# G1OJS/PyFT8

Hardware: NVIDIA B200
Metric: decoded 15-s FT8 cycles/sec (higher is better)
Workload: dtype f32

## Files before the change

### pyft8_b200/csrc/fine.cuh

```cuda
#pragma once
#include <cuda_runtime.h>
#include <stdint.h>
#include "fft.cuh"
#include "sync.cuh"

namespace ft8 {

constexpr int CS_N = 96000, CS_N1 = 375, CS_N2 = 256, CS_COLS = 16, CS_NT = 256;
constexpr int FINE_SPEC_STRIDE = 49152;
constexpr int FINE_N = 3200, FINE_NT = 256;
#define FINE_BUFS 3
constexpr int FINE_NP = FINE_N + FINE_N / 200;

template <typename T> __device__ __forceinline__ float2 load_pair(const T* x, int n);
template <> __device__ __forceinline__ float2 load_pair<int16_t>(const int16_t* x, int n) {
    const short2 v = *reinterpret_cast<const short2*>(x + 2 * n);
    return make_float2((float)v.x, (float)v.y);
}
template <> __device__ __forceinline__ float2 load_pair<float>(const float* x, int n) {
    return *reinterpret_cast<const float2*>(x + 2 * n);
}

template <typename T>
__global__ void __launch_bounds__(CS_NT)
k_cs_cols(const T* __restrict__ audio, float2* __restrict__ Y, const float2* __restrict__ TC,
          const float2* __restrict__ W96000T) {
    extern __shared__ float2 cs_smem[];
    const int cyc = blockIdx.y, n2_0 = blockIdx.x * CS_COLS;
    const T* x = audio + (size_t)cyc * CYCLE_SAMPLES;
    constexpr int LD_ITERS = (CS_COLS * CS_N1 + CS_NT - 1) / CS_NT;
#pragma unroll
    for (int b0 = 0; b0 < LD_ITERS; b0 += 8) {
        float2 v[8];
#pragma unroll
        for (int u = 0; u < 8; ++u) {
            const int i = threadIdx.x + (b0 + u) * CS_NT;
            const int n1 = i / CS_COLS, c = i - n1 * CS_COLS;
            const int n = CS_N2 * n1 + n2_0 + c;
            v[u] = (i < CS_COLS * CS_N1 && n < CYCLE_SAMPLES / 2) ? load_pair<T>(x, n) : make_float2(0.f, 0.f);
        }
#pragma unroll
        for (int u = 0; u < 8; ++u) {
            const int i = threadIdx.x + (b0 + u) * CS_NT;
            const int n1 = i / CS_COLS, c = i - n1 * CS_COLS;
            if (i < CS_COLS * CS_N1) cs_smem[c * CS_N1 + n1] = v[u];
        }
    }
    __syncthreads();
    pass_inplace_batched<375, 3, 1, CS_COLS, CS_NT, false, true>(cs_smem, threadIdx.x, TC);
    pass_inplace_batched<375, 5, 3, CS_COLS, CS_NT, false, true, true>(cs_smem, threadIdx.x, TC + 250);
    pass_inplace_batched<375, 5, 15, CS_COLS, CS_NT, false, true>(cs_smem, threadIdx.x, TC + 350);
    pass_inplace_batched<375, 5, 75, CS_COLS, CS_NT, false>(cs_smem, threadIdx.x, TC);
    float2* y = Y + (size_t)cyc * CS_N;
    for (int i = threadIdx.x; i < CS_COLS * CS_N1; i += CS_NT) {
        const int k1 = i / CS_COLS, c = i - k1 * CS_COLS;
        const int n2 = n2_0 + c;
        const float2 w = __ldg(&W96000T[k1 * CS_N2 + n2]);
        y[k1 * CS_N2 + n2] = cmul(cs_smem[c * CS_N1 + k1], w);
    }
}

constexpr int CSR_G = 8;
constexpr int CSR_STRIDE = CS_N2 + CS_N2 / 16 + 4;
__global__ void __launch_bounds__(CS_NT)
k_cs_rows(const float2* __restrict__ Y, float2* __restrict__ spec, int spec_stride, int kmax,
          const float2* __restrict__ T256, const float2* __restrict__ W192000) {
    __shared__ float2 rows[2 * CSR_G][CSR_STRIDE];
    const int cyc = blockIdx.y, g0 = blockIdx.x * CSR_G;
    const float2* y = Y + (size_t)cyc * CS_N;
    {
        float2 v[2 * CSR_G];
#pragma unroll
        for (int r = 0; r < 2 * CSR_G; ++r) {
            const int k1 = g0 + (r & (CSR_G - 1));
            const int row = (r < CSR_G) ? k1 : (CS_N1 - k1) % CS_N1;
            v[r] = (k1 <= 187) ? y[row * CS_N2 + threadIdx.x] : make_float2(0.f, 0.f);
        }
#pragma unroll
        for (int r = 0; r < 2 * CSR_G; ++r) rows[r][threadIdx.x] = v[r];
    }
    __syncthreads();
    pass_inplace_batched<256, 16, 1, 2 * CSR_G, CS_NT, false, true, false, IdMap, Pad16Map, CSR_STRIDE>(&rows[0][0], threadIdx.x, T256);
    pass_inplace_batched<256, 16, 16, 2 * CSR_G, CS_NT, false, false, false, Pad16Map, IdMap, CSR_STRIDE>(&rows[0][0], threadIdx.x, T256);
    float2* out = spec + (size_t)cyc * spec_stride;
    for (int i = threadIdx.x; i < CSR_G * CS_N2; i += CS_NT) {
        const int k2 = i / CSR_G, r = i - k2 * CSR_G;
        const int k1 = g0 + r;
        if (k1 > 187) continue;
        const int k = k1 + CS_N1 * k2;
        const int k2m = (k1 == 0) ? ((CS_N2 - k2) & (CS_N2 - 1)) : (CS_N2 - 1 - k2);
        const float2 zk = rows[r][k2];
        const float2 zm = rows[CSR_G + r][k2m];
        const float2 e = cscale(0.5f, cfma_elem(zm, 1.0f, -1.0f, zk));
        const float2 dz = cfma_elem(zm, -1.0f, 1.0f, zk);
            const float2 o = make_float2(0.5f * dz.y, -0.5f * dz.x);
        const float2 wo = cmul(o, __ldg(&W192000[k]));
        if (k <= kmax) out[k] = cadd(e, wo);
        const int km = CS_N - k;
        if (km <= kmax && !(k1 == 0 && k2 > 128)) out[km] = make_float2(e.x - wo.x, -(e.y - wo.y));
    }
}

struct FineTables {
    float taper[100];
    float2 w32[32];
};
__constant__ FineTables c_fine;

struct FineOut {
    int32_t tt, ff, nsync;
    float sd;
    int32_t snr;
};

constexpr int FINE_T5_OFF = 4 * 640, FINE_T8_OFF = FINE_T5_OFF + 4 * 128, FINE_TF_LEN = FINE_T8_OFF + 7 * 16;

struct FineIn { float2 a0[5]; float2 ax[4]; };

__device__ __forceinline__ void fine_pass12_load(FineIn& in, const float2* __restrict__ spec, int fb, int p2) {
#pragma unroll
    for (int j = 0; j < 5; ++j) in.a0[j] = __ldg(&spec[fb + p2 + 128 * j]);
    in.ax[0] = __ldg(&spec[fb + p2 + 640]);
    in.ax[1] = (p2 + 128 < 210) ? __ldg(&spec[fb + p2 + 128 + 640]) : make_float2(0.f, 0.f);
    in.ax[2] = (p2 + 384 >= 490) ? __ldg(&spec[fb + p2 + 384 - 640]) : make_float2(0.f, 0.f);
    in.ax[3] = __ldg(&spec[fb + p2 + 512 - 640]);
}

template <int Q, bool A4> __device__ __forceinline__ float2 fine_b(float2 a0, float2 ax) {
    const float2 w1 = make_float2(0.30901699437494742410f, 0.95105651629515357212f);
    const float2 w2 = make_float2(-0.80901699437494742410f, 0.58778525229247312917f);
    if (Q == 0) return cadd(a0, ax);
    const float2 w = (Q == 1 || Q == 4) ? w1 : w2;
    const bool conj = (Q >= 3) != A4;
    return cadd(a0, conj ? cmulc(ax, w) : cmul(ax, w));
}

template <int Q>
__device__ __forceinline__ void fine_pass12_col(const FineIn& in, const float2 (&ax)[4], float2* dst, int p2,
                                                const float2* __restrict__ TF, const float2 (&w)[8]) {
    float2 a[5];
    a[0] = fine_b<Q, false>(in.a0[0], ax[0]);
    a[1] = (p2 < 82) ? fine_b<Q, false>(in.a0[1], ax[1]) : in.a0[1];
    a[2] = in.a0[2];
    a[3] = (p2 >= 106) ? fine_b<Q, true>(in.a0[3], ax[2]) : in.a0[3];
    a[4] = fine_b<Q, true>(in.a0[4], ax[3]);
    if (Q > 0) {
#pragma unroll
        for (int j = 0; j < 5; ++j) a[j] = cmulc(a[j], __ldg(&TF[(Q - 1) * 640 + p2 + 128 * j]));
    }
    Dft<5, true>::run(a);
    dst[Q + 25 * p2] = a[0];
#pragma unroll
    for (int k = 1; k < 5; ++k) dst[Q + 25 * p2 + 5 * k] = cmulc(a[k], w[k - 1]);
}

__device__ __forceinline__ void fine_pass12_finish(const FineIn& in, float2* dst, int p2, const float2* __restrict__ TF,
                                                   const float* taper, const float2 (&w)[8]) {
    float2 ax[4] = {in.ax[0], in.ax[1], in.ax[2], in.ax[3]};
    if (p2 >= 110) ax[0] = cscale(taper[p2 - 110], ax[0]);
    if (p2 < 82) ax[1] = cscale(taper[p2 + 18], ax[1]);
    if (p2 >= 106) ax[2] = cscale(taper[p2 - 106], ax[2]);
    if (p2 < 78) ax[3] = cscale(taper[p2 + 22], ax[3]);
    fine_pass12_col<0>(in, ax, dst, p2, TF, w);
    fine_pass12_col<1>(in, ax, dst, p2, TF, w);
    fine_pass12_col<2>(in, ax, dst, p2, TF, w);
    fine_pass12_col<3>(in, ax, dst, p2, TF, w);
    fine_pass12_col<4>(in, ax, dst, p2, TF, w);
}

__device__ __forceinline__ void fine_pass12(float2* dst, const float2* __restrict__ spec, int fb, int p2,
                                            const float2* __restrict__ TF, const float* taper, const float2 (&w)[8]) {
    FineIn in;
    fine_pass12_load(in, spec, fb, p2);
    fine_pass12_finish(in, dst, p2, TF, taper, w);
}

template <int NT>
__device__ __forceinline__ void fine_pass3(const float2* src, float2* dst, int tid, const float2 (&tw8)[7]) {
    const int p = tid & 15;
#pragma unroll
    for (int r = 0; r < (25 * 16 + NT - 1) / NT; ++r) {
        const int q = (tid >> 4) + (NT / 16) * r;
        if (q < 25) {
            float2 a[8];
#pragma unroll
            for (int j = 0; j < 8; ++j) a[j] = src[q + 25 * p + 400 * j];
            Dft<8, true>::run(a);
            float2* d = dst + q + 201 * p;
            d[0] = a[0];
#pragma unroll
            for (int k = 1; k < 8; ++k) d[25 * k] = cmulc(a[k], tw8[k - 1]);
        }
    }
    __syncthreads();
}

template <int NT>
__device__ __forceinline__ void fine_last_full(const float2* src, float2* dst, int tid) {
#pragma unroll
    for (int t0 = 0; t0 < 200; t0 += NT) {
        const int t = t0 + tid;
        if (t < 200) {
            float2 a[16];
#pragma unroll
            for (int j = 0; j < 16; ++j) a[j] = src[t + 201 * j];
            Dft<16, true>::run(a);
#pragma unroll
            for (int k = 0; k < 16; ++k) dst[t + 200 * k] = a[k];
        }
    }
    __syncthreads();
}

__device__ __forceinline__ void fine_pass4_window(const float2* x, float2* zwin, int n0, int len, int tid, const float2* w16) {
#pragma unroll
    for (int o = tid; o < 256; o += 128) if (o < len) {
        const int n = n0 + o;
        const int kk = n / 200, q = n - 200 * kk;
        const int r = kk & 3;
        const float sg = (r & 1) ? -1.0f : 1.0f;
        const float2 ir = make_float2(r == 0 ? 1.0f : (r == 2 ? -1.0f : 0.0f), r == 1 ? 1.0f : (r == 3 ? -1.0f : 0.0f));
        float2 y[4];
#pragma unroll
        for (int b = 0; b < 4; ++b) {
            const float2 x0 = x[q + 201 * b], x1 = x[q + 201 * (4 + b)], x2 = x[q + 201 * (8 + b)], x3 = x[q + 201 * (12 + b)];
            const float2 s = caxpy(sg, x2, x0), t = caxpy(sg, x3, x1);
            y[b] = cmac(s, t, ir);
        }
        float2 acc = y[0];
#pragma unroll
        for (int b = 1; b < 4; ++b) acc = cmac(acc, y[b], w16[(b * kk) & 15]);
        zwin[o] = acc;
    }
}

__device__ __forceinline__ float2 shfl_xor2(float2 v, int o) {
    return make_float2(__shfl_xor_sync(0xffffffffu, v.x, o), __shfl_xor_sync(0xffffffffu, v.y, o));
}

__device__ __forceinline__ float dft32x4_mag(const float2* z, int i0, int lane, const float2 (&tw)[8]) {
    const int m = lane & 7;
    float2 v[4];
#pragma unroll
    for (int a = 0; a < 4; ++a) v[a] = z[i0 + m + 8 * a];
    Dft<4, false>::run(v);
    float2 c[8];
#pragma unroll
    for (int t = 0; t < 8; ++t) c[t] = cmul(v[t & 3], tw[t]);
    const bool h4 = lane & 4, h2 = lane & 2, h1 = lane & 1;
    float2 d4[4], d2[2];
#pragma unroll
    for (int j = 0; j < 4; ++j) {
        const float2 send = h4 ? c[j] : c[j + 4], keep = h4 ? c[j + 4] : c[j];
        d4[j] = cadd(keep, shfl_xor2(send, 4));
    }
#pragma unroll
    for (int j = 0; j < 2; ++j) {
        const float2 send = h2 ? d4[j] : d4[j + 2], keep = h2 ? d4[j + 2] : d4[j];
        d2[j] = cadd(keep, shfl_xor2(send, 2));
    }
    const float2 send = h1 ? d2[0] : d2[1], keep = h1 ? d2[1] : d2[0];
    const float2 s = cadd(keep, shfl_xor2(send, 1));
    return sqrtf(fmaf(s.x, s.x, s.y * s.y)) * (1.0f / 3200.0f);
}

__device__ __forceinline__ int clip_start(int i) { return max(0, min(FINE_N - 32, i)); }

__device__ __forceinline__ float costas_rows4(const float2* z, int z0, int k0, int lane, const float2 (&tw)[8]) {
    const int k = k0 + (lane >> 3), bin = lane & 7;
    const float g = dft32x4_mag(z, z0 + 32 * min(k, 6), lane, tw);
    float c = 0.0f;
    if (k < 7 && bin < 7) c = (bin == ((0x2560413 >> (4 * k)) & 7)) ? g : g * (-1.0f / 6.0f);
#pragma unroll
    for (int o = 16; o > 0; o >>= 1) c += __shfl_xor_sync(0xffffffffu, c, o);
    return c;
}

constexpr int FINE_SMEM_BYTES = (FINE_N + 2 * FINE_NP) * (int)sizeof(float2) + (79 * 8 + 16 + 100) * (int)sizeof(float) + (32 + 16 + 256) * (int)sizeof(float2);

#ifdef FINE_PROFILE
__device__ unsigned long long g_fine_prof[16];
#define FP_T(v) const long long v = clock64()
#define FP_ADD(i, d) do { if (lane == 0) atomicAdd(&g_fine_prof[i], (unsigned long long)(d)); } while (0)
#else
#define FP_T(v)
#define FP_ADD(i, d)
#endif
__global__ void __launch_bounds__(FINE_NT, 2)
k_fine(const float2* __restrict__ spec, int spec_stride, const int32_t* __restrict__ list, const int32_t* __restrict__ count,
       int n_direct, const int32_t* __restrict__ cycle_of, const int16_t* __restrict__ cand_f0,
       const int16_t* __restrict__ cand_h0, const float2* __restrict__ TF, FineOut* __restrict__ fo,
       float* __restrict__ llr_fine, float* __restrict__ sig_grid) {
    extern __shared__ float2 fine_smem[];
    float* G = reinterpret_cast<float*>(fine_smem + FINE_N + 2 * FINE_NP);
    float* score = G + 79 * 8;
    float* taper = score + 16;
    float2* w32 = reinterpret_cast<float2*>(taper + 100);
    float2* w16 = w32 + 32;
    float2* zwin = w16 + 16;
    const int tid = threadIdx.x, lane = tid & 31, warp = tid >> 5;
    if (tid < 32) w32[tid] = c_fine.w32[tid];
    if (tid < 16) { const float2 w = c_fine.w32[2 * tid]; w16[tid] = make_float2(w.x, -w.y); }
    if (tid < 100) taper[tid] = c_fine.taper[tid];
    __syncthreads();
    float2 tw[8];
#pragma unroll
    for (int t = 0; t < 8; ++t) tw[t] = w32[(t * (lane & 7)) & 31];
    if (warp >= 4) {
#pragma unroll
        for (int k = 1; k < 5; ++k) tw[k - 1] = __ldg(&TF[FINE_T5_OFF + (k - 1) * 128 + (tid - 128)]);
    }
    float2 tw8[7];
#pragma unroll
    for (int k = 1; k < 8; ++k) tw8[k - 1] = __ldg(&TF[FINE_T8_OFF + (k - 1) * 16 + (tid & 15)]);
    const int n_items = list ? *count : n_direct;
    if (warp >= 4 && (int)blockIdx.x < n_items) {
        const int slot = list ? list[blockIdx.x] : (int)blockIdx.x;
        fine_pass12(fine_smem, spec + (size_t)cycle_of[slot] * spec_stride, 50 * cand_f0[slot], tid - 128, TF, taper, tw);
    }
    __syncthreads();
    for (int item = blockIdx.x; item < n_items; item += gridDim.x) {
        const int slot = list ? list[item] : item;
        const int cyc = cycle_of[slot];
        const int f0 = cand_f0[slot], h0 = cand_h0[slot];
        const float2* sp = spec + (size_t)cyc * spec_stride;
        const int fb0 = 50 * f0;
        const int tb0 = (h0 >= 0) ? 8 * h0 : 8 * h0 + 1;
        float2 *px = fine_smem, *po = fine_smem + FINE_N, *pb = fine_smem + FINE_N + FINE_NP;
        FineIn fin;
        FP_T(ts0);
        if (warp >= 4) fine_pass12_load(fin, sp, fb0 - 32, tid - 128);
        fine_pass3<FINE_NT>(px, po, tid, tw8);
        FP_T(ts1);
        if (warp < 4) {
            fine_pass4_window(po, zwin, tb0 - 8 + 1152, 238, tid, w16);
            asm volatile("bar.sync 1, 128;" ::: "memory");
#pragma unroll
            for (int u = 0; u < 2; ++u) {
                const int st = 2 * warp + u;
                const float sc = costas_rows4(zwin, 2 * st, 0, lane, tw) + costas_rows4(zwin, 2 * st, 4, lane, tw);
                if (lane == 0) score[st] = sc;
            }
            FP_T(ts2);
            if (warp == 0) { FP_ADD(8, ts1 - ts0); FP_ADD(9, ts2 - ts1); FP_ADD(11, 1); }
        } else {
            fine_pass12_finish(fin, px, tid - 128, TF, taper, tw);
            FP_T(ts2);
            if (warp == 4) FP_ADD(10, ts2 - ts1);
        }
        __syncthreads();
        int tt = -8;
        float bestf = score[0];
        for (int ti = 1; ti < 8; ++ti) if (score[ti] > bestf) { bestf = score[ti]; tt = -8 + 2 * ti; }
        { float2* t = pb; pb = po; po = t; }
        int best_fi = 4;
        for (int e = 0; e < 8; ++e) {
            const int fi = e < 4 ? e : e + 1;
            if (warp >= 4 && e < 7) fine_pass12_load(fin, sp, fb0 + (-32 + 8 * (e + 1 < 4 ? e + 1 : e + 2)), tid - 128);
            FP_T(t0);
            fine_pass3<FINE_NT>(px, po, tid, tw8);
            FP_T(t1);
            if (warp < 4) {
                fine_pass4_window(po, zwin, tb0 + tt + 1152, 224, tid, w16);
                FP_T(tw0);
                asm volatile("bar.sync 1, 128;" ::: "memory");
                if (warp < 2) {
                    const float r = costas_rows4(zwin, 0, 4 * warp, lane, tw);
                    if (lane == 0) score[8 + warp] = r;
                }
                FP_T(t2);
                if (warp == 0) { FP_ADD(0, t1 - t0); FP_ADD(1, t2 - t1); FP_ADD(4, tw0 - t1); FP_ADD(6, 1); }
                if (warp == 3) { FP_ADD(5, t2 - t1); }
            } else if (e < 7) {
                fine_pass12_finish(fin, px, tid - 128, TF, taper, tw);
                FP_T(t2);
                if (warp == 4) { FP_ADD(2, t2 - t1); FP_ADD(7, 1); }
            }
            __syncthreads();
            FP_T(t3);
            if (warp == 0) FP_ADD(3, t3 - t1);
            const float sc = score[8] + score[9];
            if (sc > bestf || (sc == bestf && fi < best_fi)) { bestf = sc; best_fi = fi; float2* t = pb; pb = po; po = t; }
        }
        const int ff = -32 + 8 * best_fi;
        FP_T(tf0);
        fine_last_full<FINE_NT>(pb, po, tid);
        FP_T(tf1);
        if (warp < 4) {
            const float2* z = po;
            for (int j0 = 4 * warp; j0 < 79; j0 += 16) {
                const int j = j0 + (lane >> 3);
                const float g = dft32x4_mag(z, clip_start(tb0 + tt + 32 * min(j, 78)), lane, tw);
                if (j < 79) G[j * 8 + (lane & 7)] = g;
            }
            asm volatile("bar.sync 1, 128;" ::: "memory");
            if (sig_grid) for (int i = tid; i < 79 * 8; i += 128) sig_grid[(size_t)slot * 632 + i] = G[i];
            if (tid < 32) {
                int hit = 0;
                if (lane < 21) {
                    const int blk = lane / 7, k = lane - 7 * blk;
                    const int row = (blk == 0) ? k : (blk == 1 ? 36 + k : 72 + k);
                    int am = 0;
                    float mv = G[row * 8];
                    for (int t = 1; t < 8; ++t) if (G[row * 8 + t] > mv) { mv = G[row * 8 + t]; am = t; }
                    hit = (am == ((0x2560413 >> (4 * k)) & 7)) ? 1 : 0;
                }
                const int nsync = __reduce_add_sync(0xffffffffu, hit);
                float p[2][8];
                if (lane < 29) {
#pragma unroll
                    for (int q = 0; q < 2; ++q) {
                        const int sym = lane + (q ? 43 : 7);
#pragma unroll
                        for (int t = 0; t < 8; ++t) p[q][t] = 20.0f * log10f(G[sym * 8 + t]);
                    }
                }
                float sd; int snr;
                llr_from_payload_warp(p, lane, llr_fine + (size_t)slot * 174, sd, snr);
                if (lane == 0) {
                    FineOut o; o.tt = tt; o.ff = ff; o.nsync = nsync; o.sd = sd; o.snr = snr;
                    fo[slot] = o;
// ... 20 lines not shown
```

### pyft8_b200/csrc/fine_tc.cuh

```cuda
#pragma once
#include <cuda_runtime.h>
#include <stdint.h>
#include "fine.cuh"

namespace ft8 {

struct TScanOut { int32_t tt; float score0; };

constexpr int FS_WIN = 224;
constexpr int FS_CAND = 32;
constexpr int FS_K1 = 64, FS_NU = 328, FS_K = FS_K1 + FS_NU, FS_KC = 8, FS_CHUNKS = FS_K / FS_KC;
constexpr int FS_N = 64;
constexpr int FS_TILES = 4;
constexpr int FS_STAGES = 4;
constexpr int FS_ACC_COLS = FS_TILES * FS_N;
constexpr int FS_A_STAGE_COLS = FS_TILES * 16;
constexpr int FS_B_SPLIT_BYTES = 2 * FS_N * 16;
constexpr int FS_B_STAGE_BYTES = 2 * FS_B_SPLIT_BYTES;
constexpr int FS_GEN_WARPS = 16;
constexpr int FS_BSTAGES = 8;
constexpr int FS_ISSUERS = 4;
constexpr int FS_NT = (FS_GEN_WARPS + FS_ISSUERS + 1) * 32;
constexpr int FS_W_LEN = 6400;
constexpr int FS_SMEM_BYTES = FS_BSTAGES * FS_B_STAGE_BYTES + FS_W_LEN * 8;
constexpr int FS_BMAT_FLOATS = FS_CHUNKS * FS_B_STAGE_BYTES / 4;
static_assert(FS_ACC_COLS + FS_STAGES * FS_A_STAGE_COLS == 512, "TMEM column plan");

__host__ __device__ __forceinline__ int fs_u_of(int j) { return j < 164 ? j - 182 : j + 554; }

__device__ __forceinline__ uint32_t smem_u32(const void* p) { return (uint32_t)__cvta_generic_to_shared(p); }
__device__ __forceinline__ void mbar_init(uint32_t a, int count) { asm volatile("mbarrier.init.shared::cta.b64 [%0], %1;" ::"r"(a), "r"(count)); }
__device__ __forceinline__ void mbar_expect_tx(uint32_t a, int bytes) {
    asm volatile("mbarrier.arrive.expect_tx.shared::cta.b64 _, [%0], %1;" ::"r"(a), "r"(bytes) : "memory");
}
__device__ __forceinline__ void mbar_wait(uint32_t a, uint32_t parity) {
    uint32_t done = 0;
    for (uint32_t spin = 0; !done; ++spin) {
        asm volatile("{\n\t.reg .pred p;\n\tmbarrier.try_wait.parity.shared::cta.b64 p, [%1], %2;\n\tselp.u32 %0, 1, 0, p;\n\t}"
                     : "=r"(done) : "r"(a), "r"(parity) : "memory");
        if (spin > (1u << 24)) __trap();
    }
}
__device__ __forceinline__ void bulk_g2s(uint32_t dst, const void* src, int bytes, uint32_t mbar) {
    asm volatile("cp.async.bulk.shared::cluster.global.mbarrier::complete_tx::bytes [%0], [%1], %2, [%3];"
                 ::"r"(dst), "l"(src), "r"(bytes), "r"(mbar) : "memory");
}
__device__ __forceinline__ void fence_proxy_async() { asm volatile("fence.proxy.async.shared::cta;" ::: "memory"); }
__device__ __forceinline__ void tc_fence_before() { asm volatile("tcgen05.fence::before_thread_sync;" ::: "memory"); }
__device__ __forceinline__ void tc_fence_after() { asm volatile("tcgen05.fence::after_thread_sync;" ::: "memory"); }
__device__ __forceinline__ void tc_commit(uint32_t mbar) {
    asm volatile("tcgen05.commit.cta_group::1.mbarrier::arrive::one.shared::cluster.b64 [%0];" ::"r"(mbar) : "memory");
}
__device__ __forceinline__ uint64_t umma_desc(uint32_t saddr, int lbo_bytes, int sbo_bytes) {
    return (uint64_t)((saddr >> 4) & 0x3FFF) | ((uint64_t)((lbo_bytes >> 4) & 0x3FFF) << 16) | ((uint64_t)((sbo_bytes >> 4) & 0x3FFF) << 32) |
           (1ull << 46);
}
constexpr uint32_t FS_IDESC = (1u << 4) | (2u << 7) | (2u << 10) | ((FS_N >> 3) << 17) | ((128u >> 4) << 24);
__device__ __forceinline__ void umma_tf32(uint32_t d_tmem, uint64_t da, uint64_t db, uint32_t accumulate) {
    asm volatile("{\n\t.reg .pred p;\n\tsetp.ne.b32 p, %4, 0;\n\t"
                 "tcgen05.mma.cta_group::1.kind::tf32 [%0], %1, %2, %3, {%5, %5, %5, %5}, p;\n\t}"
                 ::"r"(d_tmem), "l"(da), "l"(db), "r"(FS_IDESC), "r"(accumulate), "r"(0u) : "memory");
}
__device__ __forceinline__ void tmem_ld32(uint32_t taddr, uint32_t (&v)[32]) {
    asm volatile("tcgen05.ld.sync.aligned.32x32b.x32.b32 "
                 "{%0, %1, %2, %3, %4, %5, %6, %7, %8, %9, %10, %11, %12, %13, %14, %15, "
                 "%16, %17, %18, %19, %20, %21, %22, %23, %24, %25, %26, %27, %28, %29, %30, %31}, [%32];"
                 : "=r"(v[0]), "=r"(v[1]), "=r"(v[2]), "=r"(v[3]), "=r"(v[4]), "=r"(v[5]), "=r"(v[6]), "=r"(v[7]), "=r"(v[8]), "=r"(v[9]),
                   "=r"(v[10]), "=r"(v[11]), "=r"(v[12]), "=r"(v[13]), "=r"(v[14]), "=r"(v[15]), "=r"(v[16]), "=r"(v[17]), "=r"(v[18]),
                   "=r"(v[19]), "=r"(v[20]), "=r"(v[21]), "=r"(v[22]), "=r"(v[23]), "=r"(v[24]), "=r"(v[25]), "=r"(v[26]), "=r"(v[27]),
                   "=r"(v[28]), "=r"(v[29]), "=r"(v[30]), "=r"(v[31])
                 : "r"(taddr) : "memory");
}
__device__ __forceinline__ void tmem_ld_wait() { asm volatile("tcgen05.wait::ld.sync.aligned;" ::: "memory"); }
__device__ __forceinline__ float4 ldg_v4_pinned(const void* p) {
    float4 v;
    asm volatile("ld.global.nc.v4.f32 {%0, %1, %2, %3}, [%4];" : "=f"(v.x), "=f"(v.y), "=f"(v.z), "=f"(v.w) : "l"(p));
    return v;
}
__device__ __forceinline__ float2 ldg_v2_pinned(const void* p) {
    float2 v;
    asm volatile("ld.global.nc.v2.f32 {%0, %1}, [%2];" : "=f"(v.x), "=f"(v.y) : "l"(p));
    return v;
}
__device__ __forceinline__ float tf32_hi(float x) { return __uint_as_float(__float_as_uint(x) & 0xFFFFE000u); }

struct FineItem { int slot, f0, h0, cyc, tt, ff; };

constexpr int FT_NT = 128;
constexpr int FT_CTAS = 4;
constexpr int FF_CTAS = 3;
constexpr int FT_SMEM_BYTES = (FINE_N + FINE_NP) * (int)sizeof(float2) + (16 + 100) * (int)sizeof(float) + (32 + 16 + 256) * (int)sizeof(float2);

__global__ void __launch_bounds__(FT_NT, FT_CTAS)
k_fine_tscan(const float2* __restrict__ spec, int spec_stride, const int32_t* __restrict__ list, const int32_t* __restrict__ count,
             int n_direct, const int32_t* __restrict__ cycle_of, const int16_t* __restrict__ cand_f0, const int16_t* __restrict__ cand_h0,
             const float2* __restrict__ TF, TScanOut* __restrict__ tso, float2* __restrict__ zwin_out) {
    extern __shared__ float2 fine_smem[];
    float2 *px = fine_smem, *po = fine_smem + FINE_N;
    float* score = reinterpret_cast<float*>(fine_smem + FINE_N + FINE_NP);
    float* taper = score + 16;
    float2* w32 = reinterpret_cast<float2*>(taper + 100);
    float2* w16 = w32 + 32;
    float2* zwin = w16 + 16;
    const int tid = threadIdx.x, lane = tid & 31, warp = tid >> 5;
    if (tid < 32) w32[tid] = c_fine.w32[tid];
    if (tid < 16) { const float2 w = c_fine.w32[2 * tid]; w16[tid] = make_float2(w.x, -w.y); }
    if (tid < 100) taper[tid] = c_fine.taper[tid];
    __syncthreads();
    float2 tw[8];
#pragma unroll
    for (int t = 0; t < 8; ++t) tw[t] = w32[(t * (lane & 7)) & 31];
    float2 tw5[8];
#pragma unroll
    for (int k = 1; k < 5; ++k) tw5[k - 1] = __ldg(&TF[FINE_T5_OFF + (k - 1) * 128 + (tid & 127)]);
    float2 tw8[7];
#pragma unroll
    for (int k = 1; k < 8; ++k) tw8[k - 1] = __ldg(&TF[FINE_T8_OFF + (k - 1) * 16 + (tid & 15)]);
    const int n_items = list ? *count : n_direct;
    FineItem cur{}, nxt{};
    FineIn in;
    int item = blockIdx.x;
    if (item < n_items) {
        cur.slot = list ? list[item] : item;
        cur.f0 = cand_f0[cur.slot]; cur.h0 = cand_h0[cur.slot]; cur.cyc = cycle_of[cur.slot];
        fine_pass12_load(in, spec + (size_t)cur.cyc * spec_stride, 50 * cur.f0, tid & 127);
    }
    for (; item < n_items; item += gridDim.x) {
        const int h0 = cur.h0;
        const int tb0 = (h0 >= 0) ? 8 * h0 : 8 * h0 + 1;
        const int nitem = item + gridDim.x;
        const bool nhave = nitem < n_items;
        if (nhave) nxt.slot = list ? list[nitem] : nitem;
        fine_pass12_finish(in, px, tid, TF, taper, tw5);
        __syncthreads();
        fine_pass3<FT_NT>(px, po, tid, tw8);
        if (nhave) { nxt.f0 = cand_f0[nxt.slot]; nxt.h0 = cand_h0[nxt.slot]; nxt.cyc = cycle_of[nxt.slot]; }
        {
            const int n0 = tb0 - 8 + 1152;
            for (int o = tid; o < 238; o += FT_NT) {
                const int n = n0 + o;
                const int kk = n / 200, q = n - 200 * kk;
                const int r = kk & 3;
                const float sg = (r & 1) ? -1.0f : 1.0f;
                const float2 ir = make_float2(r == 0 ? 1.0f : (r == 2 ? -1.0f : 0.0f), r == 1 ? 1.0f : (r == 3 ? -1.0f : 0.0f));
                float2 y[4];
#pragma unroll
                for (int b = 0; b < 4; ++b) {
                    const float2 x0 = po[q + 201 * b], x1 = po[q + 201 * (4 + b)], x2 = po[q + 201 * (8 + b)], x3 = po[q + 201 * (12 + b)];
                    const float2 s = caxpy(sg, x2, x0), t = caxpy(sg, x3, x1);
                    y[b] = cmac(s, t, ir);
                }
                float2 acc = y[0];
#pragma unroll
                for (int b = 1; b < 4; ++b) acc = cmac(acc, y[b], w16[(b * kk) & 15]);
                zwin[o] = acc;
            }
        }
        __syncthreads();
        if (nhave) fine_pass12_load(in, spec + (size_t)nxt.cyc * spec_stride, 50 * nxt.f0, tid & 127);
        for (int st = warp; st < 8; st += FT_NT / 32) {
            const float sc = costas_rows4(zwin, 2 * st, 0, lane, tw) + costas_rows4(zwin, 2 * st, 4, lane, tw);
            if (lane == 0) score[st] = sc;
        }
        __syncthreads();
        int tt = -8;
        float bestf = score[0];
        for (int ti = 1; ti < 8; ++ti) if (score[ti] > bestf) { bestf = score[ti]; tt = -8 + 2 * ti; }
        if (tid == 0) { TScanOut o; o.tt = tt; o.score0 = bestf; tso[item] = o; }
        for (int i = tid; i < FS_WIN; i += FT_NT) zwin_out[(size_t)item * FS_WIN + i] = zwin[tt + 8 + i];
        __syncthreads();
        cur = nxt;
    }
}

constexpr float FS_AMB_TOL = 1e-4f;

struct FsCand { int spec_off; int m0; int valid; float score0; };

#ifdef FS_PROFILE
__device__ unsigned long long g_fs_prof[16];
#define FSP_T(v) const long long v = clock64()
#define FSP_ADD(i, d) do { if (lane == 0) atomicAdd(&g_fs_prof[i], (unsigned long long)(d)); } while (0)
#else
#define FSP_T(v)
#define FSP_ADD(i, d)
#endif

__device__ __forceinline__ void mbar_arrive(uint32_t a) { asm volatile("mbarrier.arrive.shared::cta.b64 _, [%0];" ::"r"(a) : "memory"); }
__device__ __forceinline__ void umma_tf32_ts(uint32_t d_tmem, uint32_t a_tmem, uint64_t db, uint32_t accumulate) {
    asm volatile("{\n\t.reg .pred p;\n\tsetp.ne.b32 p, %4, 0;\n\t"
                 "tcgen05.mma.cta_group::1.kind::tf32 [%0], [%1], %2, %3, {%5, %5, %5, %5}, p;\n\t}"
                 ::"r"(d_tmem), "r"(a_tmem), "l"(db), "r"(FS_IDESC), "r"(accumulate), "r"(0u) : "memory");
}
__device__ __forceinline__ void tmem_st4(uint32_t taddr, float a, float b, float c, float d) {
    asm volatile("tcgen05.st.sync.aligned.32x32b.x4.b32 [%0], {%1, %2, %3, %4};"
                 ::"r"(taddr), "r"(__float_as_uint(a)), "r"(__float_as_uint(b)), "r"(__float_as_uint(c)), "r"(__float_as_uint(d)) : "memory");
}
__device__ __forceinline__ void tmem_st8(uint32_t taddr, const float (&v)[8]) {
    asm volatile("tcgen05.st.sync.aligned.32x32b.x8.b32 [%0], {%1, %2, %3, %4, %5, %6, %7, %8};"
                 ::"r"(taddr), "r"(__float_as_uint(v[0])), "r"(__float_as_uint(v[1])), "r"(__float_as_uint(v[2])), "r"(__float_as_uint(v[3])),
                   "r"(__float_as_uint(v[4])), "r"(__float_as_uint(v[5])), "r"(__float_as_uint(v[6])), "r"(__float_as_uint(v[7])) : "memory");
}
__device__ __forceinline__ void tmem_st_wait() { asm volatile("tcgen05.wait::st.sync.aligned;" ::: "memory"); }

__global__ void __launch_bounds__(FS_NT, 1)
k_fscan_mma(const float2* __restrict__ spec, int spec_stride, const int32_t* __restrict__ list, const int32_t* __restrict__ count,
            int n_direct, const int32_t* __restrict__ cycle_of, const int16_t* __restrict__ cand_f0, const int16_t* __restrict__ cand_h0,
            const TScanOut* __restrict__ tso, const float2* __restrict__ zwin, const float* __restrict__ bmat,
            const float2* __restrict__ w6400, int32_t* __restrict__ ff_out, int32_t* __restrict__ amb_list,
            int32_t* __restrict__ amb_count) {
    extern __shared__ __align__(1024) unsigned char fs_smem[];
    unsigned char* bstage = fs_smem;
    float2* W = reinterpret_cast<float2*>(fs_smem + FS_BSTAGES * FS_B_STAGE_BYTES);
    __shared__ uint64_t bars[2 * FS_STAGES + 2 * FS_BSTAGES + 2];
    __shared__ uint32_t tmem_slot;
    __shared__ FsCand s_cand[2][FS_CAND];
    __shared__ float s_score[FS_CAND][8];
    const int tid = threadIdx.x, lane = tid & 31, warp = tid >> 5;
    const uint32_t bar_a = smem_u32(&bars[0]), bar_free = smem_u32(&bars[FS_STAGES]), bar_b = smem_u32(&bars[2 * FS_STAGES]);
    const uint32_t bar_bfree = smem_u32(&bars[2 * FS_STAGES + FS_BSTAGES]);
    const uint32_t bar_acc = smem_u32(&bars[2 * FS_STAGES + 2 * FS_BSTAGES]), bar_accfree = bar_acc + 8;
    for (int i = tid; i < FS_W_LEN; i += FS_NT) W[i] = __ldg(&w6400[i]);
    if (tid == 0) {
        for (int s = 0; s < FS_STAGES; ++s) { mbar_init(bar_a + 8 * s, 4); mbar_init(bar_free + 8 * s, FS_ISSUERS); }
        for (int s = 0; s < FS_BSTAGES; ++s) { mbar_init(bar_b + 8 * s, 1); mbar_init(bar_bfree + 8 * s, FS_ISSUERS); }
        mbar_init(bar_acc, FS_ISSUERS); mbar_init(bar_accfree, FS_GEN_WARPS);
        asm volatile("fence.mbarrier_init.release.cluster;" ::: "memory");
    }
    if (warp == 0) {
        asm volatile("tcgen05.alloc.cta_group::1.sync.aligned.shared::cta.b32 [%0], 512;" ::"r"(smem_u32(&tmem_slot)) : "memory");
        asm volatile("tcgen05.relinquish_alloc_permit.cta_group::1.sync.aligned;" ::: "memory");
    }
    tc_fence_before();
    __syncthreads();
    tc_fence_after();
    const uint32_t tmem_base = tmem_slot;
    const int n_items = list ? *count : n_direct;
    const int n_pass = (n_items + FS_CAND - 1) / FS_CAND;
    const int my_passes = (int)blockIdx.x < n_pass ? (n_pass - 1 - (int)blockIdx.x) / (int)gridDim.x + 1 : 0;

    if (warp == FS_GEN_WARPS + FS_ISSUERS) {
        if (lane == 0) {
            const uint32_t total = (uint32_t)my_passes * FS_CHUNKS;
// ... 68 lines not shown
                zrow[rr] = reinterpret_cast<const float*>(zwin) + ((size_t)(pass * FS_CAND + cl0 + 16 * rr) * FS_WIN + 32 * s_sym) * 2;
                srow[rr] = spec + cd.spec_off;
                rot[rr] = W[m[rr]];
            }
            float2 cur[2][8], nxt[2][8];
            auto load_chunk = [&](int c, float2 (&d)[2][8]) {
#pragma unroll
                for (int rr = 0; rr < 2; ++rr) {
                    if (!ok[rr]) continue;
                    if (c < FS_K1 / FS_KC) {
                        const float4 a = ldg_v4_pinned(zrow[rr] + 8 * c);
                        const float4 b = ldg_v4_pinned(zrow[rr] + 8 * c + 4);
                        d[rr][0] = make_float2(a.x, a.y); d[rr][1] = make_float2(a.z, a.w);
                        d[rr][2] = make_float2(b.x, b.y); d[rr][3] = make_float2(b.z, b.w);
                    } else {
                        const int j0 = (c - FS_K1 / FS_KC) * FS_KC;
#pragma unroll
                        for (int q = 0; q < 2; ++q) {
                            const float2* p = srow[rr] + fs_u_of(j0 + 4 * q);
                            if (vec_ok) {
                                const float4 a = ldg_v4_pinned(p), b = ldg_v4_pinned(p + 2);
                                d[rr][4 * q] = make_float2(a.x, a.y); d[rr][4 * q + 1] = make_float2(a.z, a.w);
                                d[rr][4 * q + 2] = make_float2(b.x, b.y); d[rr][4 * q + 3] = make_float2(b.z, b.w);
                            } else {
#pragma unroll
                                for (int e = 0; e < 4; ++e) d[rr][4 * q + e] = ldg_v2_pinned(p + e);
                            }
                        }
                    }
                }
            };
            load_chunk(grp, cur);
            FSP_T(p0);
            for (int c = grp; c < FS_CHUNKS; c += 4) {
                FSP_T(g0);
                if (c + 4 < FS_CHUNKS) load_chunk(c + 4, nxt);
                const uint32_t it = (uint32_t)pn * FS_CHUNKS + c, st = it % FS_STAGES, use = it / FS_STAGES;
                FSP_T(g1);
                if (use >= 1) mbar_wait(bar_free + 8 * st, (use - 1) & 1);
                FSP_T(g2);
                tc_fence_after();
                const uint32_t ta = tmem_base + lane_field + FS_ACC_COLS + st * FS_A_STAGE_COLS;
#pragma unroll
                for (int rr = 0; rr < 2; ++rr) {
                    float re[8], im[8];
                    if (!ok[rr]) {
#pragma unroll
                        for (int e = 0; e < 8; ++e) { re[e] = 0.f; im[e] = 0.f; }
                    } else if (c < FS_K1 / FS_KC) {
#pragma unroll
                        for (int e = 0; e < 4; ++e) {
                            const float2 z = cur[rr][e];
                            re[2 * e] = z.x; re[2 * e + 1] = -z.y;
                            im[2 * e] = z.y; im[2 * e + 1] = z.x;
                        }
                    } else {
                        const int j0 = (c - FS_K1 / FS_KC) * FS_KC;
#pragma unroll
                        for (int q = 0; q < 2; ++q) {
                            float2 ph = W[((fs_u_of(j0 + 4 * q) + FS_W_LEN) * m[rr]) % FS_W_LEN];
#pragma unroll
                            for (int e = 0; e < 4; ++e) {
                                const float2 a = cur[rr][4 * q + e];
                                re[4 * q + e] = fmaf(a.x, ph.x, -a.y * ph.y);
                                im[4 * q + e] = fmaf(a.x, ph.y, a.y * ph.x);
                                if (e < 3) ph = make_float2(fmaf(ph.x, rot[rr].x, -ph.y * rot[rr].y), fmaf(ph.x, rot[rr].y, ph.y * rot[rr].x));
                            }
                        }
                    }
                    float hi[8], lo[8];
#pragma unroll
                    for (int e = 0; e < 8; ++e) { hi[e] = tf32_hi(re[e]); lo[e] = re[e] - hi[e]; }
                    tmem_st8(ta + 32 * rr, hi);
                    tmem_st8(ta + 32 * rr + 8, lo);
#pragma unroll
                    for (int e = 0; e < 8; ++e) { hi[e] = tf32_hi(im[e]); lo[e] = im[e] - hi[e]; }
                    tmem_st8(ta + 32 * rr + 16, hi);
                    tmem_st8(ta + 32 * rr + 24, lo);
                }
                tmem_st_wait();
                tc_fence_before();
                __syncwarp();
                if (lane == 0) mbar_arrive(bar_a + 8 * st);
                FSP_T(g3);
                if (gw == 0) { FSP_ADD(6, g1 - g0); FSP_ADD(7, g2 - g1); FSP_ADD(8, g3 - g2); FSP_ADD(9, 1); }
#pragma unroll
                for (int rr = 0; rr < 2; ++rr)
#pragma unroll
                    for (int e = 0; e < 8; ++e) cur[rr][e] = nxt[rr][e];
            }
            FSP_T(e0);
            mbar_wait(bar_acc, pn & 1);
            FSP_T(e1);
            if (gw == 0) { FSP_ADD(10, e0 - p0); FSP_ADD(11, e1 - e0); FSP_ADD(12, 1); }
            tc_fence_after();
            {
                const int epair = (gw >> 2) & 1, fh = gw >> 3;
                uint32_t vr[32], vi[32];
                tmem_ld32(tmem_base + lane_field + (2 * epair) * FS_N + 32 * fh, vr);
                tmem_ld32(tmem_base + lane_field + (2 * epair + 1) * FS_N + 32 * fh, vi);
                tmem_ld_wait();
                tc_fence_before();
                __syncwarp();
                if (lane == 0) mbar_arrive(bar_accfree);
                const int costas_t = (0x2560413 >> (4 * min(lane & 7, 6))) & 7;
                float sc[4];
#pragma unroll
                for (int f = 0; f < 4; ++f) {
                    float a = 0.f;
#pragma unroll
                    for (int t = 0; t < 7; ++t) {
                        const float x = __uint_as_float(vr[8 * f + t]), y = __uint_as_float(vi[8 * f + t]);
                        const float gmag = sqrtf(fmaf(x, x, y * y)) * (1.0f / 3200.0f);
                        a += (t == costas_t) ? gmag : gmag * (-1.0f / 6.0f);
                    }
                    a = ((lane & 7) < 7) ? a : 0.f;
                    a += __shfl_xor_sync(0xffffffffu, a, 1);
                    a += __shfl_xor_sync(0xffffffffu, a, 2);
                    a += __shfl_xor_sync(0xffffffffu, a, 4);
                    sc[f] = a;
                }
                if ((lane & 7) == 0) {
                    const int ecl = 16 * epair + 4 * (gw & 3) + (lane >> 3);
#pragma unroll
                    for (int f = 0; f < 4; ++f) s_score[ecl][4 * fh + f] = sc[f];
                }
            }
            asm volatile("bar.sync 1, %0;" ::"n"(FS_GEN_WARPS * 32) : "memory");
            if (tid < FS_CAND && sc_buf[tid].valid) {
                float bestf = sc_buf[tid].score0;
                int best_fi = 4;
                float second = -INFINITY, scale = fabsf(bestf);
#pragma unroll
                for (int e = 0; e < 8; ++e) {
                    const int fi = e < 4 ? e : e + 1;
                    const float v = s_score[tid][e];
                    scale = fmaxf(scale, fabsf(v));
                    if (v > bestf || (v == bestf && fi < best_fi)) { second = bestf; bestf = v; best_fi = fi; }
                    else second = fmaxf(second, v);
                }
                ff_out[pass * FS_CAND + tid] = -32 + 8 * best_fi;
                if (amb_list && bestf - second <= FS_AMB_TOL * scale) {
                    const int item = pass * FS_CAND + tid;
                    amb_list[atomicAdd(amb_count, 1)] = list ? list[item] : item;
                }
            }
        }
    }
    tc_fence_before();
    __syncthreads();
    if (warp == 0) asm volatile("tcgen05.dealloc.cta_group::1.sync.aligned.b32 %0, 512;" ::"r"(tmem_base) : "memory");
}

constexpr int FF_SMEM_BYTES = (FINE_N + FINE_NP) * (int)sizeof(float2) + 100 * (int)sizeof(float) + 32 * (int)sizeof(float2);

__global__ void __launch_bounds__(FT_NT, FF_CTAS)
k_fine_final(const float2* __restrict__ spec, int spec_stride, const int32_t* __restrict__ list, const int32_t* __restrict__ count,
             int n_direct, const int32_t* __restrict__ cycle_of, const int16_t* __restrict__ cand_f0, const int16_t* __restrict__ cand_h0,
             const float2* __restrict__ TF, const TScanOut* __restrict__ tso, const int32_t* __restrict__ ff_in,
             FineOut* __restrict__ fo, float* __restrict__ llr_fine, float* __restrict__ sig_grid) {
    extern __shared__ float2 fine_smem[];
    float2 *px = fine_smem, *po = fine_smem + FINE_N;
    float* G = reinterpret_cast<float*>(po);
    float* P = G + 79 * 8;
    float* taper = reinterpret_cast<float*>(fine_smem + FINE_N + FINE_NP);
    float2* w32 = reinterpret_cast<float2*>(taper + 100);
    const int tid = threadIdx.x, lane = tid & 31, warp = tid >> 5;
    if (tid < 32) w32[tid] = c_fine.w32[tid];
    if (tid < 100) taper[tid] = c_fine.taper[tid];
    __syncthreads();
    float2 tw[8];
#pragma unroll
    for (int t = 0; t < 8; ++t) tw[t] = w32[(t * (lane & 7)) & 31];
    float2 tw5[8];
#pragma unroll
    for (int k = 1; k < 5; ++k) tw5[k - 1] = __ldg(&TF[FINE_T5_OFF + (k - 1) * 128 + (tid & 127)]);
    float2 tw8[7];
#pragma unroll
    for (int k = 1; k < 8; ++k) tw8[k - 1] = __ldg(&TF[FINE_T8_OFF + (k - 1) * 16 + (tid & 15)]);
    const int n_items = list ? *count : n_direct;
    __shared__ int s_nsync;
    FineItem cur{}, nxt{};
    FineIn in;
    int item = blockIdx.x;
    if (item < n_items) {
        cur.slot = list ? list[item] : item;
        cur.f0 = cand_f0[cur.slot]; cur.h0 = cand_h0[cur.slot]; cur.cyc = cycle_of[cur.slot];
        cur.tt = tso[item].tt; cur.ff = ff_in[item];
        fine_pass12_load(in, spec + (size_t)cur.cyc * spec_stride, 50 * cur.f0 + cur.ff, tid & 127);
    }
    for (; item < n_items; item += gridDim.x) {
        const int slot = cur.slot, h0 = cur.h0, tt = cur.tt, ff = cur.ff;
        const int tb0 = (h0 >= 0) ? 8 * h0 : 8 * h0 + 1;
        const int nitem = item + gridDim.x;
        const bool nhave = nitem < n_items;
        if (nhave) { nxt.slot = list ? list[nitem] : nitem; nxt.tt = tso[nitem].tt; nxt.ff = ff_in[nitem]; }
        fine_pass12_finish(in, px, tid, TF, taper, tw5);
        __syncthreads();
        fine_pass3<FT_NT>(px, po, tid, tw8);
        if (nhave) { nxt.f0 = cand_f0[nxt.slot]; nxt.h0 = cand_h0[nxt.slot]; nxt.cyc = cycle_of[nxt.slot]; }
        fine_last_full<FT_NT>(po, px, tid);
        if (nhave) fine_pass12_load(in, spec + (size_t)nxt.cyc * spec_stride, 50 * nxt.f0 + nxt.ff, tid & 127);
        for (int gi = warp; gi < 6; gi += FT_NT / 32) {
            const int i = 4 * gi + (lane >> 3), ii = min(i, 20);
            const int row = 36 * (ii / 7) + ii % 7;
            const float g = dft32x4_mag(px, clip_start(tb0 + tt + 32 * row), lane, tw);
            if (i < 21) G[row * 8 + (lane & 7)] = g;
        }
        __syncthreads();
        if (warp == 0) {
            int hit = 0;
            if (lane < 21) {
                const int blk = lane / 7, k = lane - 7 * blk;
                const int row = 36 * blk + k;
                int am = 0;
                float mv = G[row * 8];
                for (int t = 1; t < 8; ++t) if (G[row * 8 + t] > mv) { mv = G[row * 8 + t]; am = t; }
                hit = (am == ((0x2560413 >> (4 * k)) & 7)) ? 1 : 0;
            }
            const int ns = __reduce_add_sync(0xffffffffu, hit);
            if (lane == 0) s_nsync = ns;
        }
        __syncthreads();
        const int nsync = s_nsync;
        const bool full = sig_grid != nullptr || nsync > 6;
        if (full) {
            for (int gi = warp; gi < 15; gi += FT_NT / 32) {
                const int r = 4 * gi + (lane >> 3), rr = min(r, 57);
                const int sym = rr < 29 ? rr + 7 : rr + 14;
                const float g = dft32x4_mag(px, clip_start(tb0 + tt + 32 * sym), lane, tw);
                if (r < 58) { G[sym * 8 + (lane & 7)] = g; P[r * 8 + (lane & 7)] = 20.0f * log10f(g); }
            }
        }
        __syncthreads();
        if (sig_grid) for (int i = tid; i < 79 * 8; i += FT_NT) sig_grid[(size_t)slot * 632 + i] = G[i];
        if (warp == 0) {
            if (full) {
                float p[2][8];
                if (lane < 29) {
#pragma unroll
                    for (int q = 0; q < 2; ++q)
#pragma unroll
                        for (int t = 0; t < 8; ++t) p[q][t] = P[(lane + 29 * q) * 8 + t];
                }
                float sd; int snr;
                llr_from_payload_warp(p, lane, llr_fine + (size_t)slot * 174, sd, snr);
                if (lane == 0) { FineOut o; o.tt = tt; o.ff = ff; o.nsync = nsync; o.sd = sd; o.snr = snr; fo[slot] = o; }
            } else if (lane == 0) {
                FineOut o; o.tt = tt; o.ff = ff; o.nsync = nsync; o.sd = 0.0f; o.snr = 0; fo[slot] = o;
            }
        }
        __syncthreads();
        cur = nxt;
    }
}

}
```

Before: 71040.

## Run fine-final FFT in a single padded in-place buffer to raise occupancy

The k_fine_final kernel now does its 3200-point FFT in one padded shared buffer, in place, instead of ping-ponging between two buffers. Pass 1/2 writes directly into the padded layout and the DFT readers index with a stride-201 pad. Twiddle tables are now looked up from shared or global memory through small accessor structs rather than held in register arrays. The software prefetch of the next item's spectrum is dropped and the launch bound rises from 3 to 6 CTAs per SM, trading less load latency hiding for more resident blocks. There is a risk of races: the trailing __syncthreads at the end of each loop iteration was removed while the next item immediately overwrites buf.

```diff
diff --git a/pyft8_b200/csrc/fine.cuh b/pyft8_b200/csrc/fine.cuh
--- a/pyft8_b200/csrc/fine.cuh
+++ b/pyft8_b200/csrc/fine.cuh
@@ -135,9 +135,9 @@
     return cadd(a0, conj ? cmulc(ax, w) : cmul(ax, w));
 }
 
-template <int Q>
+template <int Q, bool PAD = false, typename W5>
 __device__ __forceinline__ void fine_pass12_col(const FineIn& in, const float2 (&ax)[4], float2* dst, int p2,
-                                                const float2* __restrict__ TF, const float2 (&w)[8]) {
+                                                const float2* __restrict__ TF, const W5& w) {
     float2 a[5];
     a[0] = fine_b<Q, false>(in.a0[0], ax[0]);
     a[1] = (p2 < 82) ? fine_b<Q, false>(in.a0[1], ax[1]) : in.a0[1];
@@ -149,30 +149,33 @@
         for (int j = 0; j < 5; ++j) a[j] = cmulc(a[j], __ldg(&TF[(Q - 1) * 640 + p2 + 128 * j]));
     }
     Dft<5, true>::run(a);
-    dst[Q + 25 * p2] = a[0];
-#pragma unroll
-    for (int k = 1; k < 5; ++k) dst[Q + 25 * p2 + 5 * k] = cmulc(a[k], w[k - 1]);
-}
-
+    float2* d = dst + (PAD ? Q + 25 * (p2 >> 4) + 201 * (p2 & 15) : Q + 25 * p2);
+    d[0] = a[0];
+#pragma unroll
+    for (int k = 1; k < 5; ++k) d[5 * k] = cmulc(a[k], w[k - 1]);
+}
+
+template <bool PAD = false, typename W5>
 __device__ __forceinline__ void fine_pass12_finish(const FineIn& in, float2* dst, int p2, const float2* __restrict__ TF,
-                                                   const float* taper, const float2 (&w)[8]) {
+                                                   const float* taper, const W5& w) {
     float2 ax[4] = {in.ax[0], in.ax[1], in.ax[2], in.ax[3]};
     if (p2 >= 110) ax[0] = cscale(taper[p2 - 110], ax[0]);
     if (p2 < 82) ax[1] = cscale(taper[p2 + 18], ax[1]);
     if (p2 >= 106) ax[2] = cscale(taper[p2 - 106], ax[2]);
     if (p2 < 78) ax[3] = cscale(taper[p2 + 22], ax[3]);
-    fine_pass12_col<0>(in, ax, dst, p2, TF, w);
-    fine_pass12_col<1>(in, ax, dst, p2, TF, w);
-    fine_pass12_col<2>(in, ax, dst, p2, TF, w);
-    fine_pass12_col<3>(in, ax, dst, p2, TF, w);
-    fine_pass12_col<4>(in, ax, dst, p2, TF, w);
-}
-
+    fine_pass12_col<0, PAD>(in, ax, dst, p2, TF, w);
+    fine_pass12_col<1, PAD>(in, ax, dst, p2, TF, w);
+    fine_pass12_col<2, PAD>(in, ax, dst, p2, TF, w);
+    fine_pass12_col<3, PAD>(in, ax, dst, p2, TF, w);
+    fine_pass12_col<4, PAD>(in, ax, dst, p2, TF, w);
+}
+
+template <bool PAD = false, typename W5>
 __device__ __forceinline__ void fine_pass12(float2* dst, const float2* __restrict__ spec, int fb, int p2,
-                                            const float2* __restrict__ TF, const float* taper, const float2 (&w)[8]) {
+                                            const float2* __restrict__ TF, const float* taper, const W5& w) {
     FineIn in;
     fine_pass12_load(in, spec, fb, p2);
-    fine_pass12_finish(in, dst, p2, TF, taper, w);
+    fine_pass12_finish<PAD>(in, dst, p2, TF, taper, w);
 }
 
 template <int NT>
@@ -195,7 +198,7 @@
     __syncthreads();
 }
 
-template <int NT>
+template <int NT, int OS = 200>
 __device__ __forceinline__ void fine_last_full(const float2* src, float2* dst, int tid) {
 #pragma unroll
     for (int t0 = 0; t0 < 200; t0 += NT) {
@@ -206,7 +209,7 @@
             for (int j = 0; j < 16; ++j) a[j] = src[t + 201 * j];
             Dft<16, true>::run(a);
 #pragma unroll
-            for (int k = 0; k < 16; ++k) dst[t + 200 * k] = a[k];
+            for (int k = 0; k < 16; ++k) dst[t + OS * k] = a[k];
         }
     }
     __syncthreads();
@@ -238,11 +241,15 @@
     return make_float2(__shfl_xor_sync(0xffffffffu, v.x, o), __shfl_xor_sync(0xffffffffu, v.y, o));
 }
 
-__device__ __forceinline__ float dft32x4_mag(const float2* z, int i0, int lane, const float2 (&tw)[8]) {
+template <bool PAD = false, typename TW>
+__device__ __forceinline__ float dft32x4_mag(const float2* z, int i0, int lane, const TW& tw) {
     const int m = lane & 7;
     float2 v[4];
 #pragma unroll
-    for (int a = 0; a < 4; ++a) v[a] = z[i0 + m + 8 * a];
+    for (int a = 0; a < 4; ++a) {
+        const int n = i0 + m + 8 * a;
+        v[a] = z[PAD ? n + n / 200 : n];
+    }
     Dft<4, false>::run(v);
     float2 c[8];
 #pragma unroll
@@ -264,9 +271,16 @@
     return sqrtf(fmaf(s.x, s.x, s.y * s.y)) * (1.0f / 3200.0f);
 }
 
+struct W32Lane {
+    const float2* w32;
+    int m;
+    __device__ __forceinline__ float2 operator[](int t) const { return w32[(t * m) & 31]; }
+};
+
 __device__ __forceinline__ int clip_start(int i) { return max(0, min(FINE_N - 32, i)); }
 
-__device__ __forceinline__ float costas_rows4(const float2* z, int z0, int k0, int lane, const float2 (&tw)[8]) {
+template <typename TW>
+__device__ __forceinline__ float costas_rows4(const float2* z, int z0, int k0, int lane, const TW& tw) {
     const int k = k0 + (lane >> 3), bin = lane & 7;
     const float g = dft32x4_mag(z, z0 + 32 * min(k, 6), lane, tw);
     float c = 0.0f;
diff --git a/pyft8_b200/csrc/fine_tc.cuh b/pyft8_b200/csrc/fine_tc.cuh
--- a/pyft8_b200/csrc/fine_tc.cuh
+++ b/pyft8_b200/csrc/fine_tc.cuh
@@ -88,7 +88,6 @@
 
 constexpr int FT_NT = 128;
 constexpr int FT_CTAS = 4;
-constexpr int FF_CTAS = 3;
 constexpr int FT_SMEM_BYTES = (FINE_N + FINE_NP) * (int)sizeof(float2) + (16 + 100) * (int)sizeof(float) + (32 + 16 + 256) * (int)sizeof(float2);
 
 __global__ void __launch_bounds__(FT_NT, FT_CTAS)
@@ -463,7 +462,39 @@
     if (warp == 0) asm volatile("tcgen05.dealloc.cta_group::1.sync.aligned.b32 %0, 512;" ::"r"(tmem_base) : "memory");
 }
 
-constexpr int FF_SMEM_BYTES = (FINE_N + FINE_NP) * (int)sizeof(float2) + 100 * (int)sizeof(float) + 32 * (int)sizeof(float2);
+constexpr int FF_CTAS = 6;
+
+template <typename T8>
+__device__ __forceinline__ void fine_pass3_inplace(float2* buf, int tid, const T8& tw8) {
+    const int p = tid & 15;
+#pragma unroll
+    for (int r = 0; r < (25 * 16 + FT_NT - 1) / FT_NT; ++r) {
+        const int q = (tid >> 4) + (FT_NT / 16) * r;
+        if (q < 25) {
+            float2* d = buf + q + 201 * p;
+            float2 a[8];
+#pragma unroll
+            for (int j = 0; j < 8; ++j) a[j] = d[25 * j];
+            Dft<8, true>::run(a);
+            d[0] = a[0];
+#pragma unroll
+            for (int k = 1; k < 8; ++k) d[25 * k] = cmulc(a[k], tw8[k - 1]);
+        }
+    }
+}
+
+struct T5Ldg {
+    const float2* TF;
+    int p2;
+    __device__ __forceinline__ float2 operator[](int i) const { return __ldg(&TF[FINE_T5_OFF + i * 128 + p2]); }
+};
+struct T8Lane {
+    const float2* t8;
+    int p;
+    __device__ __forceinline__ float2 operator[](int i) const { return t8[i * 16 + p]; }
+};
+
+constexpr int FF_SMEM_BYTES = FINE_NP * (int)sizeof(float2) + (79 * 8 + 58 * 8 + 100 + 2) * (int)sizeof(float) + (32 + 7 * 16) * (int)sizeof(float2);
 
 __global__ void __launch_bounds__(FT_NT, FF_CTAS)
 k_fine_final(const float2* __restrict__ spec, int spec_stride, const int32_t* __restrict__ list, const int32_t* __restrict__ count,
@@ -471,51 +502,39 @@
              const float2* __restrict__ TF, const TScanOut* __restrict__ tso, const int32_t* __restrict__ ff_in,
              FineOut* __restrict__ fo, float* __restrict__ llr_fine, float* __restrict__ sig_grid) {
     extern __shared__ float2 fine_smem[];
-    float2 *px = fine_smem, *po = fine_smem + FINE_N;
-    float* G = reinterpret_cast<float*>(po);
+    float2* buf = fine_smem;
+    float* G = reinterpret_cast<float*>(fine_smem + FINE_NP);
     float* P = G + 79 * 8;
-    float* taper = reinterpret_cast<float*>(fine_smem + FINE_N + FINE_NP);
-    float2* w32 = reinterpret_cast<float2*>(taper + 100);
+    float* taper = P + 58 * 8;
+    int* s_nsync = reinterpret_cast<int*>(taper + 100);
+    float2* w32 = reinterpret_cast<float2*>(s_nsync + 2);
+    float2* t8 = w32 + 32;
     const int tid = threadIdx.x, lane = tid & 31, warp = tid >> 5;
     if (tid < 32) w32[tid] = c_fine.w32[tid];
     if (tid < 100) taper[tid] = c_fine.taper[tid];
+    if (tid < 7 * 16) t8[tid] = __ldg(&TF[FINE_T8_OFF + tid]);
     __syncthreads();
-    float2 tw[8];
-#pragma unroll
-    for (int t = 0; t < 8; ++t) tw[t] = w32[(t * (lane & 7)) & 31];
-    float2 tw5[8];
-#pragma unroll
-    for (int k = 1; k < 5; ++k) tw5[k - 1] = __ldg(&TF[FINE_T5_OFF + (k - 1) * 128 + (tid & 127)]);
-    float2 tw8[7];
-#pragma unroll
-    for (int k = 1; k < 8; ++k) tw8[k - 1] = __ldg(&TF[FINE_T8_OFF + (k - 1) * 16 + (tid & 15)]);
+    const W32Lane tw{w32, lane & 7};
+    const T5Ldg tw5{TF, tid};
+    const T8Lane tw8{t8, tid & 15};
     const int n_items = list ? *count : n_direct;
-    __shared__ int s_nsync;
-    FineItem cur{}, nxt{};
-    FineIn in;
-    int item = blockIdx.x;
-    if (item < n_items) {
-        cur.slot = list ? list[item] : item;
-        cur.f0 = cand_f0[cur.slot]; cur.h0 = cand_h0[cur.slot]; cur.cyc = cycle_of[cur.slot];
-        cur.tt = tso[item].tt; cur.ff = ff_in[item];
-        fine_pass12_load(in, spec + (size_t)cur.cyc * spec_stride, 50 * cur.f0 + cur.ff, tid & 127);
-    }
-    for (; item < n_items; item += gridDim.x) {
-        const int slot = cur.slot, h0 = cur.h0, tt = cur.tt, ff = cur.ff;
+    for (int item = blockIdx.x; item < n_items; item += gridDim.x) {
+        {
+            const int slot = list ? list[item] : item;
+            fine_pass12<true>(buf, spec + (size_t)cycle_of[slot] * spec_stride, 50 * cand_f0[slot] + ff_in[item], tid, TF, taper, tw5);
+        }
+        __syncthreads();
+        fine_pass3_inplace(buf, tid, tw8);
+        __syncthreads();
+        fine_last_full<FT_NT, 201>(buf, buf, tid);
+        const int slot = list ? list[item] : item;
+        const int tt = tso[item].tt, ff = ff_in[item];
+        const int h0 = cand_h0[slot];
         const int tb0 = (h0 >= 0) ? 8 * h0 : 8 * h0 + 1;
-        const int nitem = item + gridDim.x;
-        const bool nhave = nitem < n_items;
-        if (nhave) { nxt.slot = list ? list[nitem] : nitem; nxt.tt = tso[nitem].tt; nxt.ff = ff_in[nitem]; }
-        fine_pass12_finish(in, px, tid, TF, taper, tw5);
-        __syncthreads();
-        fine_pass3<FT_NT>(px, po, tid, tw8);
-        if (nhave) { nxt.f0 = cand_f0[nxt.slot]; nxt.h0 = cand_h0[nxt.slot]; nxt.cyc = cycle_of[nxt.slot]; }
-        fine_last_full<FT_NT>(po, px, tid);
-        if (nhave) fine_pass12_load(in, spec + (size_t)nxt.cyc * spec_stride, 50 * nxt.f0 + nxt.ff, tid & 127);
         for (int gi = warp; gi < 6; gi += FT_NT / 32) {
             const int i = 4 * gi + (lane >> 3), ii = min(i, 20);
             const int row = 36 * (ii / 7) + ii % 7;
-            const float g = dft32x4_mag(px, clip_start(tb0 + tt + 32 * row), lane, tw);
+            const float g = dft32x4_mag<true>(buf, clip_start(tb0 + tt + 32 * row), lane, tw);
             if (i < 21) G[row * 8 + (lane & 7)] = g;
         }
         __syncthreads();
@@ -530,16 +549,16 @@
                 hit = (am == ((0x2560413 >> (4 * k)) & 7)) ? 1 : 0;
             }
             const int ns = __reduce_add_sync(0xffffffffu, hit);
-            if (lane == 0) s_nsync = ns;
-        }
-        __syncthreads();
-        const int nsync = s_nsync;
+            if (lane == 0) *s_nsync = ns;
+        }
+        __syncthreads();
+        const int nsync = *s_nsync;
         const bool full = sig_grid != nullptr || nsync > 6;
         if (full) {
             for (int gi = warp; gi < 15; gi += FT_NT / 32) {
                 const int r = 4 * gi + (lane >> 3), rr = min(r, 57);
                 const int sym = rr < 29 ? rr + 7 : rr + 14;
-                const float g = dft32x4_mag(px, clip_start(tb0 + tt + 32 * sym), lane, tw);
+                const float g = dft32x4_mag<true>(buf, clip_start(tb0 + tt + 32 * sym), lane, tw);
                 if (r < 58) { G[sym * 8 + (lane & 7)] = g; P[r * 8 + (lane & 7)] = 20.0f * log10f(g); }
             }
         }
@@ -561,9 +580,7 @@
                 FineOut o; o.tt = tt; o.ff = ff; o.nsync = nsync; o.sd = 0.0f; o.snr = 0; fo[slot] = o;
             }
         }
-        __syncthreads();
-        cur = nxt;
-    }
-}
-
-}
+    }
+}
+
+}
```

Result: no change. 71200, median of 6 (+0.2%).
